# facebookresearch/iris

Hardware: AMD Instinct MI355X
Metric: bake_shading throughput (shading samples/s: secondary rays traced and shaded) (higher is better)
Workload: dtype f32; 1 GPU; bake_shading train-view sequence (15 views evenly spaced among 32 cameras on a circle, one view per step), 1920x1080, SPP=128 per lobe, lobes=[0, 1, 2, 3, 4, 5, 6] (0=diffuse,1-6=specular), synthetic room seed=1 1000990 triangles, SLF H=256, Philox uniforms; pixels_per_view=2073600

## Files before the change

### include/iris_hip_debug.h

```cpp
#ifndef IRIS_HIP_DEBUG_H
#define IRIS_HIP_DEBUG_H

#include "iris_hip.h"

#ifdef __cplusplus
extern "C" {
#endif

IRIS_API int iris_debug_scene_create(const float *verts, int64_t nv, const int32_t *faces, int64_t nf, int device, int layout,
                            iris_scene **out);

enum { IRIS_BAKE_AUTO = 0, IRIS_BAKE_PIXEL_PER_WAVE = 1, IRIS_BAKE_TILE_SORTED = 2 };

IRIS_API int iris_debug_bake_diffuse(const iris_scene *, const iris_emitter *, const iris_slf *, const float *pos, const float *nrm,
                            int64_t P, int spp, const float *u2, uint64_t seed, uint32_t stream_id, const int32_t *pix_id,
                            float *Ld, int64_t *tri_next, int64_t *src_next, uint64_t *stats, int variant, void *workspace,
                            uint64_t workspace_bytes, iris_stream_t);
IRIS_API int iris_debug_bake_specular(const iris_scene *, const iris_emitter *, const iris_slf *, const float *pos, const float *nrm,
                             const float *wo, float roughness, int64_t P, int spp, const float *u2, uint64_t seed,
                             uint32_t stream_id, const int32_t *pix_id, float *Ls0, float *Ls1, int64_t *tri_next, int64_t *src_next,
                             uint64_t *stats, int variant, void *workspace, uint64_t workspace_bytes, iris_stream_t);

IRIS_API int iris_debug_set(const char *key, long long value);
IRIS_API int iris_debug_ngp_encode(const iris_ngp *, const float *position, int64_t N, uint32_t *feat, iris_stream_t);
IRIS_API const char *iris_debug_build_flags(void);
IRIS_API const char *iris_debug_source_hash(void);

#ifdef __cplusplus
}
#endif
#endif
```

### iris_amd/_lib.py

```python
import ctypes as C
import os

import torch

_HERE = os.path.dirname(os.path.abspath(__file__))
LIB_PATH = os.environ.get("IRIS_HIP_LIB") or os.path.join(_HERE, "libiris_hip.so")

BVH_DEFAULT, BVH4_F32, BVH4_Q8 = 0, 1, 3
BAKE_AUTO, BAKE_PIXEL_PER_WAVE, BAKE_TILE_SORTED = 0, 1, 2


class IrisError(RuntimeError):
    pass


class SceneInfo(C.Structure):
    _fields_ = [("n_vertices", C.c_int64), ("n_triangles", C.c_int64), ("layout", C.c_int32), ("n_nodes", C.c_int32),
                ("node_bytes", C.c_int32), ("tri_bytes", C.c_int32), ("depth", C.c_int32), ("n_leaf_records", C.c_int32),
                ("sah_cost", C.c_float), ("build_seconds", C.c_float)]


_P, _I64, _I32, _F, _D, _U64, _U32 = C.c_void_p, C.c_int64, C.c_int, C.c_float, C.c_double, C.c_uint64, C.c_uint32

PROTOTYPES = {
# ... 10 lines not shown
    "iris_emitter_destroy": [_P],
    "iris_raygen_real": [_P, _P, _I32, _I32, _I32, _P, _P, _P, _P, _P],
    "iris_raygen_synthetic": [_F, _P, _I32, _I32, _I32, _P, _P, _P, _P, _P],
    "iris_intersect": [_P, _P, _P, _I64, _P, _P, _P, _P, _P, _P],
    "iris_sample_diffuse": [_P, _P, _I64, _P, _P, _P, _P],
    "iris_sample_specular": [_P, _P, _P, _F, _I64, _P, _P, _P, _P, _P],
    "iris_sample_specular_v": [_P, _P, _P, _P, _I64, _P, _P, _P, _P, _P],
    "iris_slf_lookup": [_P, _P, _I64, _P, _P, _P],
    "iris_eval_emitter": [_P, _P, _P, _P, _P, _F, _I64, _P, _P, _P, _P],
    "iris_bake_workspace_bytes": [_I64, _I32, _I32],
    "iris_bake_diffuse": [_P, _P, _P, _P, _P, _I64, _I32, _P, _U64, _U32, _P, _P, _P, _P, _U64, _P],
    "iris_bake_specular": [_P, _P, _P, _P, _P, _P, _F, _I64, _I32, _P, _U64, _U32, _P, _P, _P, _P, _P, _U64, _P],
    "iris_debug_bake_diffuse": [_P, _P, _P, _P, _P, _I64, _I32, _P, _U64, _U32, _P, _P, _P, _P, _P, _I32, _P, _U64, _P],
    "iris_debug_bake_specular": [_P, _P, _P, _P, _P, _P, _F, _I64, _I32, _P, _U64, _U32, _P, _P, _P, _P, _P, _P, _I32, _P, _U64, _P],
    "iris_debug_set": [C.c_char_p, C.c_longlong],
    "iris_debug_build_flags": [],
    "iris_debug_source_hash": [],
    "iris_bake_view": [_P, _P, _P, _P, _P, _P, _P, _I64, _I32, _P, _P, _P, _U64, _P, _P, _P, _U64, _P],
    "iris_lerp_specular": [_P, _P, _I64, _I32, _P, _P],
    "iris_unstripe_maps": [_P, _I32, _I32, _I64, _I32, _I32, _I32, _P, _P],
    "iris_get_normal_space": [_P, _I64, _P, _P],
    "iris_double_sided": [_P, _P, _I64, _P],
    "iris_angle2xyz": [_P, _P, _I64, _P, _P],
    "iris_ggx_terms": [_I32, _P, _P, _P, _I64, _P, _P, _P],
    "iris_philox_u2": [_U64, _U64, _U32, _I64, _P, _P],
    "iris_ngp_n_params": [],
    "iris_ngp_create": [_P, _I64, C.c_double, C.c_double, C.c_int, _P],
    "iris_ngp_forward": [_P, _P, _I64, _P, _P, _P, _P],
    "iris_ngp_set_params_dev": [_P, _P, _I64, _P],
    "iris_ngp_backward_workspace_bytes": [_I64],
# ... 168 lines not shown
```

### iris_amd/bake_shading.py

```python
import math
import os
import time

import torch

from . import _lib as L
from .utils.path_tracing import ray_intersect

SPP_DIFFUSE = 256
SPPS_SPECULAR = [64, 128, 128, 128, 128, 128]
N_ROUGHNESS = 6


def roughness_levels():
    return torch.linspace(0.02, 1.0, N_ROUGHNESS)


def _common(scene, emitter, position, normal, spp, u2, pix_id, want_tri):
    position = L.require_gpu(position, torch.float32, "position").reshape(-1, 3)
    normal = L.require_gpu(normal, torch.float32, "normal").reshape(-1, 3)
    P = position.shape[0]
    dev = position.device
    if u2 is not None:
        u2 = L.require_gpu(u2, torch.float32, "u2").reshape(-1, 2)
# ... 68 lines not shown
    levels = roughness_levels().tolist()
    if stream_ids is None:
        stream_ids = [0 if r is None else 1 + min(range(N_ROUGHNESS), key=lambda k: abs(levels[k] - float(r))) for r in roughness]
    outs0 = [torch.empty(P, 3, device=dev, dtype=torch.float32) for _ in range(n)]
    outs1 = [None if roughness[l] is None else torch.empty(P, 3, device=dev, dtype=torch.float32) for l in range(n)]
    rough = (C.c_float * n)(*[-1.0 if r is None else float(r) for r in roughness])
    spp_a = (C.c_int32 * n)(*[int(s) for s in spps])
    sid = (C.c_uint32 * n)(*[int(s) for s in stream_ids])
    p0 = (C.c_void_p * n)(*[t.data_ptr() for t in outs0])
    p1 = (C.c_void_p * n)(*[None if t is None else t.data_ptr() for t in outs1])
    ws, ws_bytes = _workspace(P, 1, True, L.BAKE_AUTO, dev)
    with torch.cuda.device(dev):
        L.check(L.lib().iris_bake_view(scene.handle, emitter.handle(dev), emitter.slf.handle(dev), L.ptr(position), L.ptr(normal), L.ptr(wo), L.ptr(pix_id),
                                       P, n, rough, spp_a, sid, int(seed), p0, p1, L.ptr(ws), ws_bytes, L.stream()))
    return [outs0[l] if roughness[l] is None else (outs0[l], outs1[l]) for l in range(n)]


def view_seed(seed, im_id):
    return (int(seed) + int(im_id) * 0x9E3779B97F4A7C15) & 0xFFFFFFFFFFFFFFFF


class LobeStreams:

    def __init__(self, device, n=3, emitter=None):
        self.main = torch.cuda.current_stream(device)
        if emitter is not None:
            emitter.handle(device); emitter.slf.handle(device)
        self.side = [torch.cuda.Stream(device=device) for _ in range(n)] if n > 1 else []
        self.k = 0

# ... 253 lines not shown
```

### iris_amd/csrc/iris_bake.h

```cpp
#pragma once
#include "iris_tile.h"

namespace iris {

struct BakeArgs {
    SceneDev sc; EmitDev em; SlfDev slf;
    const float* pos; const float* nrm; const float* wo;
    const float* u2; const int32_t* pix_id;
    int64_t P; int spp; uint64_t seed; uint32_t stream_id; float rough;
    float* out0; float* out1; int64_t* tri_next;
    int64_t* src_next;
    unsigned long long* stats;
    uint32_t* stack_ovf;
    float4* scratch;
    unsigned int* tile_counter;
    int tile_px;
};

#ifndef IRIS_TILE_RAYS
#define IRIS_TILE_RAYS 5120
#endif
constexpr int kTileRays = IRIS_TILE_RAYS;

__device__ __forceinline__ void reduce_geometry(int spp, int& lpp, int& ppw, int& rounds) {
// ... 143 lines not shown
        if (pvalid && sl == 0) {
            st3(a.out0 + p * 3, mk3(a0x * inv_spp, a0y * inv_spp, a0z * inv_spp));
            if (SPEC) st3(a.out1 + p * 3, mk3(a1x * inv_spp, a1y * inv_spp, a1z * inv_spp));
        }
    }
    flush_stats<COUNT>(a, ts, n_rays);
}

#ifndef IRIS_TILE_WAVES
#define IRIS_TILE_WAVES 7
#endif
#ifndef IRIS_TILE_STACK
#define IRIS_TILE_STACK 12
#endif

template <bool SPEC, bool COUNT, int LAYOUT, int TILE_STACK>
__device__ __forceinline__ void tile_body(const BakeArgs& a, int64_t p0, int np, float4* res, uint16_t* s_sorted, uint32_t* s_stack, int* s_chunk,
                                          uint32_t* ovf, TraceStats& ts, uint32_t& n_rays) {
    const int tid = threadIdx.x, lane = tid & 63, wave = tid >> 6;
    const int spp = a.spp;
    float2* res_g = reinterpret_cast<float2*>(res + kTileRays);
    int lpp, ppw, rounds;
    reduce_geometry(spp, lpp, ppw, rounds);
    const int sub = lane / lpp, sl = lane - sub * lpp;
    const float inv_spp = 1.0f / (float)spp;
    const int nr = np * spp;
    const bool resolve = !a.em.emit_ord && !a.tri_next;
    const bool skip_dead = dead_samples_skippable(a);

    const uint32_t spp_m = spp > 1 ? (uint32_t)(0x100000000ull / (uint64_t)(uint32_t)spp) + 1u : 0u;
    auto div_spp = [&](int r) -> int { return spp > 1 ? (int)__umulhi((uint32_t)r, spp_m) : r; };

    constexpr int kFrameOff = (kTileRays + 2 * 256 * 4) / 4, kFramePx = (TILE_STACK * kBlock - kFrameOff) / 6;
    float* s_frames = reinterpret_cast<float*>(s_stack) + kFrameOff;
    const bool frames = np <= kFramePx;
    if (frames) {
        for (int pl = tid; pl < np; pl += kBlock) {
            f3 t, b;
            normal_space(ld3(a.nrm + (p0 + pl) * 3), t, b);
            float* f = s_frames + pl * 6;
            f[0] = t.x; f[1] = t.y; f[2] = t.z; f[3] = b.x; f[4] = b.y; f[5] = b.z;
        }
        __syncthreads();
    }

    tile_sort_trace<LAYOUT, COUNT, kTileRays, TILE_STACK, true, SPEC && !COUNT>(
        a.sc, nr, s_sorted, s_stack, s_chunk, ovf, ts,
        [&](int r) -> uint32_t {
            const int pl = div_spp(r), s = r - pl * spp;
            const int64_t p = p0 + pl;
            const f3 n = ld3(a.nrm + p * 3), w = SPEC ? ld3(a.wo + p * 3) : mk3(0.f, 0.f, 1.f);
            const uint64_t base = (uint64_t)(a.pix_id ? (int64_t)a.pix_id[p] : p) * (uint64_t)spp;
            f3 t, b;
            if (frames) { const float* f = s_frames + pl * 6; t = mk3(f[0], f[1], f[2]); b = mk3(f[3], f[4], f[5]); }
            else normal_space(n, t, b);
            f3 wi; float g0, g1;
            sample_lobe<SPEC>(a, p, s, n, w, t, b, base, wi, g0, g1);
            if (SPEC) res_g[r] = make_float2(g1, g0);
            const bool dead = SPEC && !COUNT && skip_dead && g0 == 0.f && g1 == 0.f;
            res[r] = dead ? make_float4(0.f, 0.f, __int_as_float(resolve ? 0 : -1), __int_as_float(resolve ? -2 : 0)) : make_float4(wi.x, wi.y, wi.z, 0.f);
            return dead ? kDeadRay : dir_bin(wi);
        },
        [&](int r, f3& o, f3& d) {
            const int64_t p = p0 + div_spp(r);
            o = ld3(a.pos + p * 3);
            const float4 qa = res[r];
            d = mk3(qa.x, qa.y, qa.z);
        },
        [&](f3& o, f3& d) { o = mk3(o.x + kRayEps * d.x, o.y + kRayEps * d.y, o.z + kRayEps * d.z); },
        [&](int r, const Hit& h) {
            if (resolve) {
                float4 q = make_float4(0.f, 0.f, 0.f, __int_as_float(-2));
                if (h.slot >= 0) {
                    const float4* tr = a.sc.tris + (int64_t)h.slot * 4;
                    const float4 tx = tr[0], ty = tr[1], tz = tr[2];
                    const float ow = tr[3].x;
                    const f3 pn = hit_position(h, mk3(tx.x, ty.x, tz.x), mk3(tx.y, ty.y, tz.y), mk3(tx.z, ty.z, tz.z));
                    q = make_float4(pn.x, pn.y, pn.z, ow);
                }
                res[r] = q;
            } else
            res[r] = make_float4(h.u, h.v, __int_as_float(h.slot), 0.f);
            if (COUNT) n_rays++; }
        );

    const int n_groups = (np + ppw - 1) / ppw;
    IRIS_PHASE_BEGIN();
    for (int g = wave; g < n_groups; g += kBlock / 64) {
        const int pl = g * ppw + sub;
        const bool pvalid = pl < np;
        float a0x = 0.f, a0y = 0.f, a0z = 0.f, a1x = 0.f, a1y = 0.f, a1z = 0.f;
        if (resolve) {
            for (int rr = 0; rr < rounds; rr += 2) {
                const int s0 = rr * 64 + sl, s1 = s0 + 64;
                const bool ok0 = pvalid && s0 < spp, ok1 = pvalid && rr + 1 < rounds && s1 < spp;
                float4 q0 = make_float4(0.f, 0.f, 0.f, __int_as_float(-2)), q1 = q0;
                float2 w0 = make_float2(0.f, 0.f), w1 = w0;
                if (ok0) { q0 = res[pl * spp + s0]; if (SPEC) w0 = res_g[pl * spp + s0]; }
                if (ok1) { q1 = res[pl * spp + s1]; if (SPEC) w1 = res_g[pl * spp + s1]; }
                const int o0 = __float_as_int(q0.w), o1 = __float_as_int(q1.w);
                int j0 = -1, j1 = -1;
                if (o0 == -1) j0 = slf_index(a.slf, mk3(q0.x, q0.y, q0.z));
                if (o1 == -1) j1 = slf_index(a.slf, mk3(q1.x, q1.y, q1.z));
                float4 r0 = make_float4(0.f, 0.f, 0.f, 0.f), r1 = r0;
                if (o0 >= 0 || j0 >= 0) r0 = *(o0 >= 0 ? a.em.radiance + o0 : a.slf.radiance + j0);
                if (o1 >= 0 || j1 >= 0) r1 = *(o1 >= 0 ? a.em.radiance + o1 : a.slf.radiance + j1);
                if (ok0) {
                    const float z = o0 >= 0 ? -0.f : 0.f;
                    const f3 Le = mk3(z + r0.x, z + r0.y, z + r0.z);
                    if (a.src_next) a.src_next[(p0 + pl) * spp + s0] = o0 >= 0 ? -2 - o0 : j0;
                    if (SPEC) { a0x += Le.x * w0.y; a0y += Le.y * w0.y; a0z += Le.z * w0.y; a1x += Le.x * w0.x; a1y += Le.y * w0.x; a1z += Le.z * w0.x; }
                    else { a0x += Le.x; a0y += Le.y; a0z += Le.z; }
                }
                if (ok1) {
                    const float z = o1 >= 0 ? -0.f : 0.f;
                    const f3 Le = mk3(z + r1.x, z + r1.y, z + r1.z);
                    if (a.src_next) a.src_next[(p0 + pl) * spp + s1] = o1 >= 0 ? -2 - o1 : j1;
                    if (SPEC) { a0x += Le.x * w1.y; a0y += Le.y * w1.y; a0z += Le.z * w1.y; a1x += Le.x * w1.x; a1y += Le.y * w1.x; a1z += Le.z * w1.x; }
                    else { a0x += Le.x; a0y += Le.y; a0z += Le.z; }
                }
            }
        } else
        for (int rr = 0; rr < rounds; ++rr) {
            const int s = rr * 64 + sl;
            if (pvalid && s < spp) {
                const float4 qa = res[pl * spp + s];
                Hit h; h.u = qa.x; h.v = qa.y; h.slot = __float_as_int(qa.z); h.t = 0.f; h.id = 0;
                f3 pn = mk3(0.f, 0.f, 0.f);
                int64_t tri = -1;
                int ord_rec = -1;
                if (h.slot >= 0) {
                    const float4* tr = a.sc.tris + (int64_t)h.slot * 4;
                    const float4 tx = tr[0], ty = tr[1], tz = tr[2];
                    if (!a.em.emit_ord) ord_rec = __float_as_int(tr[3].x);
                    pn = hit_position(h, mk3(tx.x, ty.x, tz.x), mk3(tx.y, ty.y, tz.y), mk3(tx.z, ty.z, tz.z));
                    tri = __float_as_int(tx.w);
                }
                if (a.tri_next) a.tri_next[(p0 + pl) * spp + s] = tri;
                float epdf; bool vn; int src;
                const f3 Le = eval_emitter1(a.em, a.slf, pn, tri, true, 1.0f, 0.0f, epdf, vn, src, ord_rec);
                if (a.src_next) a.src_next[(p0 + pl) * spp + s] = src;
                if (SPEC) {
                    const float2 qb = res_g[pl * spp + s];
                    a0x += Le.x * qb.y; a0y += Le.y * qb.y; a0z += Le.z * qb.y;
                    a1x += Le.x * qb.x; a1y += Le.y * qb.x; a1z += Le.z * qb.x;
                } else { a0x += Le.x; a0y += Le.y; a0z += Le.z; }
            }
        }
        for (int m = 1; m < lpp; m <<= 1) {
            a0x += __shfl_xor(a0x, m); a0y += __shfl_xor(a0y, m); a0z += __shfl_xor(a0z, m);
            if (SPEC) { a1x += __shfl_xor(a1x, m); a1y += __shfl_xor(a1y, m); a1z += __shfl_xor(a1z, m); }
        }
        if (pvalid && sl == 0) {
            const int64_t p = p0 + pl;
            st3(a.out0 + p * 3, mk3(a0x * inv_spp, a0y * inv_spp, a0z * inv_spp));
            if (SPEC) st3(a.out1 + p * 3, mk3(a1x * inv_spp, a1y * inv_spp, a1z * inv_spp));
        }
    }
    IRIS_PHASE_MARK(3);
}

constexpr int kTileChunk = 64;
__device__ __forceinline__ long long claim_tile(unsigned int* counters, long long n_tiles) {
    constexpr int kChunk = kTileChunk;
    const long long n_chunks = (n_tiles + kChunk - 1) / kChunk;
    for (int k = 0; k < 8; ++k) {
        const int x = ((int)blockIdx.x + k) & 7;
        const long long per = (n_chunks + 7 - x) / 8;
        for (;;) {
            const unsigned int c = atomicAdd(counters + x, 1u);
            const long long ch = (long long)(c / kChunk);
            if (ch >= per) break;
            const long long t = (ch * 8 + x) * kChunk + (c % kChunk);
            if (t < n_tiles) return t;
// ... 32 lines not shown
constexpr int kMaxLobes = 8;
struct ViewLobe { float rough; int spp; uint32_t stream_id; int spec; int tile_px; int tiles_per_span; float* out0; float* out1; };
struct ViewArgs {
    BakeArgs base;
    int n_lobes;
    int span_px;
    long long n_tiles;
    ViewLobe lobe[kMaxLobes];
};

template <int LAYOUT>
__global__ __launch_bounds__(kBlock, IRIS_TILE_WAVES) void bake_view_kernel(ViewArgs v) {
    constexpr int kTileStack = IRIS_TILE_STACK;
    __shared__ uint16_t s_sorted[kTileRays];
    __shared__ uint32_t s_stack[kTileStack * kBlock];
    __shared__ int s_tile, s_chunk;
    static_assert(kTileStack * kBlock * 4 >= kTileRays + 2 * 256 * 4, "stack region too small to alias the sort keys");
    const int tid = threadIdx.x;
    float4* res = v.base.scratch + (size_t)blockIdx.x * kTileRays * 2;
    uint32_t* ovf = v.base.stack_ovf + (size_t)blockIdx.x * (kStackCapacity - kTileStack) * kBlock;
    for (;;) {
        __syncthreads();
        if (tid == 0) { s_tile = (int)claim_tile(v.base.tile_counter, v.n_tiles); s_chunk = 0; }
        (s_stack + kTileRays / 4)[tid] = 0;
        __syncthreads();
        const long long vt = s_tile;
        if (vt >= v.n_tiles) break;
        const long long g = vt / kTileChunk, q = g >> 3;
        const int j = (int)(vt % kTileChunk), l = (int)(q % v.n_lobes);
        const int64_t span0 = ((q / v.n_lobes) * 8 + (g & 7)) * (int64_t)v.span_px;
        const int64_t p0 = span0 + (int64_t)j * v.lobe[l].tile_px;
        if (j >= v.lobe[l].tiles_per_span || p0 >= v.base.P) continue;
        const int np = (int)min((int64_t)v.lobe[l].tile_px, min(v.base.P, span0 + v.span_px) - p0);
        BakeArgs a = v.base;
        a.spp = v.lobe[l].spp; a.rough = v.lobe[l].rough; a.stream_id = v.lobe[l].stream_id; a.tile_px = v.lobe[l].tile_px;
        a.out0 = v.lobe[l].out0; a.out1 = v.lobe[l].out1; a.u2 = nullptr; a.tri_next = nullptr; a.src_next = nullptr;
        TraceStats ts; uint32_t n_rays = 0;
        if (v.lobe[l].spec) tile_body<true, false, LAYOUT, kTileStack>(a, p0, np, res, s_sorted, s_stack, &s_chunk, ovf, ts, n_rays);
        else tile_body<false, false, LAYOUT, kTileStack>(a, p0, np, res, s_sorted, s_stack, &s_chunk, ovf, ts, n_rays);
    }
}

}
```

### iris_amd/csrc/iris_hip.hip

```cpp
#include <hip/hip_runtime.h>

#include <chrono>
#include <cmath>
#include <cstdio>
#include <cstring>
#include <atomic>
#include <cstdlib>
#include <memory>
#include <mutex>
#include <string>
#include <vector>

#include "../../include/iris_hip.h"
#include "../../include/iris_hip_debug.h"
#include "bvh_build.h"
#include "iris_device.h"
#include "iris_trace.h"
#include "iris_bake.h"
#include "iris_pt.h"
#include "iris_cache.h"
#include "iris_denoise.h"
#include "iris_ngp.h"
#include "iris_prop.h"
#include "iris_crf.h"
// ... 23 lines not shown
    DevBuf(DevBuf&& o) noexcept : p(o.p) { o.p = nullptr; }
    DevBuf& operator=(DevBuf&& o) noexcept { std::swap(p, o.p); return *this; }
    ~DevBuf() { if (p) (void)hipFree(p); }
    hipError_t alloc(size_t bytes) { return hipMalloc(&p, bytes); }
    hipError_t upload(const void* host, size_t bytes) { return hipMemcpy(p, host, bytes, hipMemcpyHostToDevice); }
};
struct DevEvent {
    hipEvent_t ev = nullptr;
    DevEvent() = default;
    DevEvent(DevEvent&& o) noexcept : ev(o.ev) { o.ev = nullptr; }
    DevEvent& operator=(DevEvent&& o) noexcept { std::swap(ev, o.ev); return *this; }
    ~DevEvent() { if (ev) (void)hipEventDestroy(ev); }
    hipError_t create() { return hipEventCreateWithFlags(&ev, hipEventDisableTiming); }
};

static long long g_opt_bvh_tri_cost_x100 = -1, g_opt_bvh_max_leaf = -1, g_opt_phase_min = -1, g_opt_tile_target_rays = -1, g_opt_tiles_per_block = -1, g_opt_pt_tile_min = -1, g_opt_bvh_presplit_x10 = -1, g_opt_joint_max_rays = -1, g_opt_prop_bwd_targets = -1, g_opt_prop_lds_members = -1;
extern "C" IRIS_API int iris_debug_set(const char* key, long long value) {
    if (!key) return fail(IRIS_ERR_ARG, "iris_debug_set: null key");
    const std::string k(key);
    if (k == "bvh_max_leaf") g_opt_bvh_max_leaf = value;
    else if (k == "bvh_tri_cost_x100") g_opt_bvh_tri_cost_x100 = value;
    else if (k == "bvh_presplit_x10") g_opt_bvh_presplit_x10 = value;
    else if (k == "phase_min") g_opt_phase_min = value;
    else if (k == "tile_target_rays") g_opt_tile_target_rays = value;
    else if (k == "tiles_per_block") g_opt_tiles_per_block = value;
    else if (k == "pt_tile_min") g_opt_pt_tile_min = value;
    else if (k == "joint_max_rays") g_opt_joint_max_rays = value;
    else if (k == "prop_bwd_targets") g_opt_prop_bwd_targets = value;
    else if (k == "prop_lds_members") g_opt_prop_lds_members = value;
    else return fail(IRIS_ERR_ARG, "iris_debug_set: unknown option " + k);
    return IRIS_OK;
}
extern "C" IRIS_API const char* iris_version(void) { return "iris_hip 0.1 (gfx950)"; }
#ifndef IRIS_NO_FUSED_RECORDS
#define IRIS_NO_FUSED_RECORDS 0
#endif
#ifndef IRIS_BUILD_FLAGS
#define IRIS_BUILD_FLAGS "unknown"
#endif
extern "C" IRIS_API const char* iris_debug_build_flags(void) { return IRIS_BUILD_FLAGS; }
#ifndef IRIS_SOURCE_HASH
#define IRIS_SOURCE_HASH "unknown"
#endif
extern "C" IRIS_API const char* iris_debug_source_hash(void) { return IRIS_SOURCE_HASH; }
// ... 1010 lines not shown
    if (em->fused.size() >= 2) { em->retired.push_back(std::move(em->fused.front())); em->fused.erase(em->fused.begin()); }
    int prev = 0;
    if (hipGetDevice(&prev) != hipSuccess || hipSetDevice(sc->device) != hipSuccess) { (void)hipGetLastError(); return nullptr; }
    DevBuf d; DevEvent ev;
    const int64_t n_rec = (int64_t)sc->dev.n_tris + 1;
    bool ok = d.alloc((size_t)n_rec * kLeafRecordBytes) == hipSuccess && ev.create() == hipSuccess;
    if (ok) {
        hipLaunchKernelGGL(fuse_ord_kernel, dim3(grid_for(n_rec, 256, 4096)), dim3(256), 0, st, sc->dev.tris, em->dev.emit_ord, n_rec, (float4*)d.p);
        ok = hipGetLastError() == hipSuccess && hipEventRecord(ev.ev, st) == hipSuccess;
    }
    (void)hipSetDevice(prev);
    if (!ok) { (void)hipGetLastError(); return nullptr; }
    em->fused.push_back({sc->uid, std::move(d), std::move(ev), false});
    return (const float4*)em->fused.back().d_tris.p;
}
extern "C" IRIS_API int iris_bake_view(const iris_scene* sc, const iris_emitter* em, const iris_slf* slf, const float* pos, const float* nrm,
                              const float* wo, const int32_t* pix_id, int64_t P, int n_lobes, const float* roughness, const int32_t* spp,
                              const uint32_t* stream_ids, uint64_t seed, float* const* out0, float* const* out1, void* workspace,
                              uint64_t workspace_bytes, iris_stream_t stream) {
    if (!sc || !em || !slf || P < 0 || n_lobes < 1 || n_lobes > kMaxLobes || !roughness || !spp || !stream_ids || !out0 || !out1 ||
        (P > 0 && (!pos || !nrm || !wo)))
        return fail(IRIS_ERR_ARG, "iris_bake_view: bad arguments");
    if (em->dev.nf != sc->info.n_triangles)
        return fail(IRIS_ERR_ARG, "iris_bake_view: the emitter tables were built for a mesh with a different number of triangles than the scene");
    if (P == 0) return IRIS_OK;
    const uint64_t need = iris_bake_workspace_bytes(P, 1, 1);
    if (!workspace || workspace_bytes < need) return fail(IRIS_ERR_ARG, "iris_bake_view: workspace of iris_bake_workspace_bytes() bytes required");
    ViewArgs v{};
    v.base.sc = sc->dev; v.base.em = em->dev; v.base.slf = slf->dev;
    if (const float4* ft = fused_tris(sc, em, (hipStream_t)stream)) { v.base.sc.tris = ft; v.base.em.emit_ord = nullptr; }
    v.base.pos = pos; v.base.nrm = nrm; v.base.wo = wo; v.base.pix_id = pix_id; v.base.P = P; v.base.seed = seed;
    v.base.tile_counter = (unsigned int*)workspace;
    v.base.scratch = (float4*)((char*)workspace + 256);
    v.base.stack_ovf = (uint32_t*)((char*)workspace + need - stack_ovf_bytes());
    v.n_lobes = n_lobes;
    const int blocks = bake_grid_blocks();
    long long t = 0;
    int tile_px_min = kTileRays;
    for (int l = 0; l < n_lobes; ++l) {
        if (spp[l] < 1 || spp[l] > kTileRays) return fail(IRIS_ERR_ARG, "iris_bake_view: spp must be in [1, iris_bake_tile_max_spp()]");
        if (!out0[l] || (roughness[l] >= 0.f && !out1[l])) return fail(IRIS_ERR_ARG, "iris_bake_view: null output");
        int tile_px = tile_pixels(spp[l]);
        const int64_t even = (P * n_lobes + (int64_t)blocks * 4 - 1) / ((int64_t)blocks * 4);
        if (even < tile_px) tile_px = (int)std::max<int64_t>(even, std::min(tile_px, 16));
        if (tile_px < 1) tile_px = 1;
        v.lobe[l].rough = roughness[l]; v.lobe[l].spp = spp[l]; v.lobe[l].stream_id = stream_ids[l]; v.lobe[l].spec = roughness[l] >= 0.f ? 1 : 0;
        v.lobe[l].tile_px = tile_px; v.lobe[l].out0 = out0[l]; v.lobe[l].out1 = out1[l];
        tile_px_min = std::min(tile_px_min, tile_px);
        t += (P + tile_px - 1) / tile_px;
    }
    v.span_px = kTileChunk * tile_px_min;
    for (int l = 0; l < n_lobes; ++l) v.lobe[l].tiles_per_span = (v.span_px + v.lobe[l].tile_px - 1) / v.lobe[l].tile_px;
    const long long n_spans = (P + v.span_px - 1) / v.span_px;
    hipStream_t st = (hipStream_t)stream;
    v.n_tiles = ((n_spans + 7) / 8) * 8 * n_lobes * kTileChunk;
    HIP_TRY(hipMemsetAsync(workspace, 0, 256, st));
    const int grid = (int)std::min<long long>(blocks, t);
    with_layout(v.base.sc, [&](auto t) { hipLaunchKernelGGL(bake_view_kernel<decltype(t)::layout>, dim3(grid), dim3(kBlock), 0, st, v); });
    HIP_TRY(hipGetLastError());
    return IRIS_OK;
}
extern "C" IRIS_API int iris_bake_diffuse(const iris_scene* sc, const iris_emitter* em, const iris_slf* slf, const float* pos, const float* nrm,
                                 int64_t P, int spp, const float* u2, uint64_t seed, uint32_t stream_id, const int32_t* pix_id,
                                 float* Ld, int64_t* tri_next, void* workspace, uint64_t workspace_bytes, iris_stream_t stream) {
    return bake_launch(false, sc, em, slf, pos, nrm, nullptr, -1.f, P, spp, u2, seed, stream_id, pix_id, Ld, nullptr, tri_next, nullptr, nullptr,
                       IRIS_BAKE_AUTO, workspace, workspace_bytes, stream);
}
extern "C" IRIS_API int iris_bake_specular(const iris_scene* sc, const iris_emitter* em, const iris_slf* slf, const float* pos, const float* nrm,
                                  const float* wo, float roughness, int64_t P, int spp, const float* u2, uint64_t seed,
                                  uint32_t stream_id, const int32_t* pix_id, float* Ls0, float* Ls1, int64_t* tri_next,
// ... 403 lines not shown
```

### iris_amd/csrc/iris_tile.h

```cpp
#pragma once
#include "iris_trace.h"

namespace iris {

#ifndef IRIS_PRIO_A
#define IRIS_PRIO_A 0
#endif
#ifndef IRIS_PRIO_C
#define IRIS_PRIO_C 3
#endif
#ifndef IRIS_PRIO_D
#define IRIS_PRIO_D 0
#endif

__device__ __forceinline__ uint32_t dir_bin(f3 d) {
    const float ax = fabsf(d.x), ay = fabsf(d.y), az = fabsf(d.z);
    const float inv = __builtin_amdgcn_rcpf(ax + ay + az + 1e-30f);
    const float a = ax * inv, b = ay * inv;
    const float v = b * __builtin_amdgcn_rcpf(1.f - a + 1e-30f);
    const int iu = min(7, (int)(a * 8.f)), iv0 = min(3, (int)(v * 4.f));
    const int iv = (iu & 1) ? 3 - iv0 : iv0;
    const uint32_t oct = (d.x < 0.f ? 1u : 0u) | (d.y < 0.f ? 2u : 0u) | (d.z < 0.f ? 4u : 0u);
    return (oct << 5) | ((uint32_t)iu << 2) | (uint32_t)iv;
}

#ifdef IRIS_PHASE_TIMING
__device__ unsigned long long g_phase_cycles[8];
#define IRIS_PHASE_BEGIN() unsigned long long t_phase_ = clock64()
#define IRIS_PHASE_MARK(k) do { if (threadIdx.x == 0) { const unsigned long long t_ = clock64(); atomicAdd(&g_phase_cycles[k], t_ - t_phase_); t_phase_ = t_; } } while (0)
#else
#define IRIS_PHASE_BEGIN()
#define IRIS_PHASE_MARK(k)
#endif

constexpr uint32_t kDeadRay = 256u;
template <int LAYOUT, bool COUNT, int CAP, int TILE_STACK, bool GLOBAL_OVF, bool SKIP_DEAD = false, class PhaseA, class FetchRay, class Prepare, class Retire>
__device__ __forceinline__ void tile_sort_trace(const SceneDev& sc, int nr, uint16_t* s_sorted, uint32_t* s_stack, int* s_chunk, uint32_t* ovf,
                                                TraceStats& ts, PhaseA phase_a, FetchRay fetch_ray, Prepare prepare, Retire retire) {
    static_assert(TILE_STACK * kBlock * 4 >= CAP + 2 * 256 * 4, "stack region too small to alias the sort keys");
    static_assert(!SKIP_DEAD || CAP <= 32 * kBlock, "one bit per ray of a thread");
    uint8_t* s_keys = reinterpret_cast<uint8_t*>(s_stack);
    uint32_t* s_hist = s_stack + CAP / 4;
    uint32_t* s_cur = s_hist + 256;
    const int tid = threadIdx.x, lane = tid & 63, wave = tid >> 6;
    IRIS_PHASE_BEGIN();
    __builtin_amdgcn_s_setprio(IRIS_PRIO_A);
    uint32_t dead = 0;
    if (SKIP_DEAD) {
        uint32_t bit = 1u;
        for (int r = tid; r < nr; r += kBlock, bit <<= 1) {
            const uint32_t key = phase_a(r);
            if (key == kDeadRay) dead |= bit;
            else { s_keys[r] = (uint8_t)key; atomicAdd(&s_hist[key], 1u); }
        }
    } else
    for (int r = tid; r < nr; r += kBlock) {
        const uint32_t key = phase_a(r);
        s_keys[r] = (uint8_t)key;
        atomicAdd(&s_hist[key], 1u);
    }
    __syncthreads();
    IRIS_PHASE_MARK(0);
    if (wave == 0) {
        uint32_t c0 = s_hist[lane * 4], c1 = s_hist[lane * 4 + 1], c2 = s_hist[lane * 4 + 2], c3 = s_hist[lane * 4 + 3];
        uint32_t tot = c0 + c1 + c2 + c3, inc = tot;
        for (int m = 1; m < 64; m <<= 1) { uint32_t v = __shfl_up(inc, m); if (lane >= m) inc += v; }
        uint32_t ex = inc - tot;
        if (SKIP_DEAD) {
            const uint32_t first = (uint32_t)nr - (uint32_t)__builtin_amdgcn_readlane((int)inc, 63);
            ex += first;
            if (lane == 0) *s_chunk = (int)first;
        }
        s_cur[lane * 4] = ex; s_cur[lane * 4 + 1] = ex + c0; s_cur[lane * 4 + 2] = ex + c0 + c1; s_cur[lane * 4 + 3] = ex + c0 + c1 + c2;
    }
    __syncthreads();
    if (SKIP_DEAD) {
        for (int r = tid; r < nr; r += kBlock, dead >>= 1) {
            if (dead & 1u) continue;
            const uint32_t pos = atomicAdd(&s_cur[s_keys[r]], 1u);
            s_sorted[pos] = (uint16_t)r;
        }
    } else
    for (int r = tid; r < nr; r += kBlock) {
        const uint32_t pos = atomicAdd(&s_cur[s_keys[r]], 1u);
        s_sorted[pos] = (uint16_t)r;
    }
    __syncthreads();
    IRIS_PHASE_MARK(1);
    {
        int my_r = 0;
// ... 8 lines not shown
            fetch_ray(my_r, o, d);
            return true;
        };
        auto ret = [&](const Hit& h) { retire(my_r, h); };
        __builtin_amdgcn_s_setprio(IRIS_PRIO_C);
        uint32_t tid_c = threadIdx.x;
        asm volatile("" : "+v"(tid_c));
        SceneDev sc_c = sc;
        asm volatile("" : "+s"(sc_c.nodes), "+s"(sc_c.tris), "+s"(sc_c.oct_stride));
        trace_stream<LAYOUT, COUNT, TILE_STACK, GLOBAL_OVF>(sc_c, s_stack + tid_c, tid_c, ovf, &ts, fetch, prepare, ret);
        __builtin_amdgcn_s_setprio(IRIS_PRIO_D);
        IRIS_PHASE_MARK(4);
    }
    __syncthreads();
    IRIS_PHASE_MARK(2);
}

}
```

Measured before the change: 10280 Mrays/s.

## Compact live specular samples into slots and grow specular tiles by dead share

For specular lobes in the fused bake_view kernel, dead samples (zero GGX weights) are no longer given slots in the tile buffer. Live samples are compacted into slots through a per-wave ballot and prefix count, and a per-64-ray group mask maps sample indices back to those slots during shading. Because fewer slots are used, the host planner enlarges each specular tile according to a roughness-based dead-share table, up to twice the base size. If a tile ends up with more live samples than the buffer holds, the block reprocesses it as two half tiles. This is meant to cut per-tile overhead and raise the number of useful rays per tile, at the cost of overflow retries and extra indirection.

```diff
diff --git a/include/iris_hip_debug.h b/include/iris_hip_debug.h
--- a/include/iris_hip_debug.h
+++ b/include/iris_hip_debug.h
@@ -22,6 +22,8 @@
                              uint64_t *stats, int variant, void *workspace, uint64_t workspace_bytes, iris_stream_t);
 
 IRIS_API int iris_debug_set(const char *key, long long value);
+IRIS_API int iris_debug_bake_view_plan(int64_t P, int n_lobes, const float *roughness, const int32_t *spp, int blocks, int32_t *tile_px,
+                              int32_t *tiles_per_span, int32_t *span_px, int64_t *n_tiles, uint64_t *slab_bytes);
 IRIS_API int iris_debug_ngp_encode(const iris_ngp *, const float *position, int64_t N, uint32_t *feat, iris_stream_t);
 IRIS_API const char *iris_debug_build_flags(void);
 IRIS_API const char *iris_debug_source_hash(void);
diff --git a/iris_amd/_lib.py b/iris_amd/_lib.py
--- a/iris_amd/_lib.py
+++ b/iris_amd/_lib.py
@@ -48,6 +48,7 @@
     "iris_debug_bake_diffuse": [_P, _P, _P, _P, _P, _I64, _I32, _P, _U64, _U32, _P, _P, _P, _P, _P, _I32, _P, _U64, _P],
     "iris_debug_bake_specular": [_P, _P, _P, _P, _P, _P, _F, _I64, _I32, _P, _U64, _U32, _P, _P, _P, _P, _P, _P, _I32, _P, _U64, _P],
     "iris_debug_set": [C.c_char_p, C.c_longlong],
+    "iris_debug_bake_view_plan": [_I64, _I32, _P, _P, _I32, _P, _P, _P, _P, _P],
     "iris_debug_build_flags": [],
     "iris_debug_source_hash": [],
     "iris_bake_view": [_P, _P, _P, _P, _P, _P, _P, _I64, _I32, _P, _P, _P, _U64, _P, _P, _P, _U64, _P],
diff --git a/iris_amd/bake_shading.py b/iris_amd/bake_shading.py
--- a/iris_amd/bake_shading.py
+++ b/iris_amd/bake_shading.py
@@ -106,6 +106,17 @@
         L.check(L.lib().iris_bake_view(scene.handle, emitter.handle(dev), emitter.slf.handle(dev), L.ptr(position), L.ptr(normal), L.ptr(wo), L.ptr(pix_id),
                                        P, n, rough, spp_a, sid, int(seed), p0, p1, L.ptr(ws), ws_bytes, L.stream()))
     return [outs0[l] if roughness[l] is None else (outs0[l], outs1[l]) for l in range(n)]
+
+
+def view_tile_plan(P, roughness, spps, blocks=0):
+    import ctypes as C
+    n = len(roughness)
+    rough = (C.c_float * n)(*[-1.0 if r is None else float(r) for r in roughness])
+    spp_a = (C.c_int32 * n)(*[int(s) for s in spps])
+    tile_px, tps = (C.c_int32 * n)(), (C.c_int32 * n)()
+    span, n_tiles, slab = C.c_int32(), C.c_int64(), C.c_uint64()
+    L.check(L.lib().iris_debug_bake_view_plan(int(P), n, rough, spp_a, int(blocks), tile_px, tps, C.byref(span), C.byref(n_tiles), C.byref(slab)))
+    return {"tile_px": list(tile_px), "tiles_per_span": list(tps), "span_px": span.value, "n_tiles": n_tiles.value, "slab_bytes": slab.value}
 
 
 def view_seed(seed, im_id):
diff --git a/iris_amd/csrc/iris_bake.h b/iris_amd/csrc/iris_bake.h
--- a/iris_amd/csrc/iris_bake.h
+++ b/iris_amd/csrc/iris_bake.h
@@ -181,9 +181,11 @@
 #define IRIS_TILE_STACK 12
 #endif
 
-template <bool SPEC, bool COUNT, int LAYOUT, int TILE_STACK>
-__device__ __forceinline__ void tile_body(const BakeArgs& a, int64_t p0, int np, float4* res, uint16_t* s_sorted, uint32_t* s_stack, int* s_chunk,
-                                          uint32_t* ovf, TraceStats& ts, uint32_t& n_rays) {
+constexpr int kLiveTileSamples = 2 * kTileRays;
+template <bool SPEC, bool COUNT, int LAYOUT, int TILE_STACK, bool LIVE = false>
+__device__ __forceinline__ bool tile_body(const BakeArgs& a, int64_t p0, int np, float4* res, uint16_t* s_sorted, uint32_t* s_stack, int* s_chunk,
+                                          uint32_t* ovf, TraceStats& ts, uint32_t& n_rays, int* s_nlive = nullptr) {
+    static_assert(!LIVE || (SPEC && !COUNT), "live slots: specular production tiles only");
     const int tid = threadIdx.x, lane = tid & 63, wave = tid >> 6;
     const int spp = a.spp;
     float2* res_g = reinterpret_cast<float2*>(res + kTileRays);
@@ -193,7 +195,8 @@
     const float inv_spp = 1.0f / (float)spp;
     const int nr = np * spp;
     const bool resolve = !a.em.emit_ord && !a.tri_next;
-    const bool skip_dead = dead_samples_skippable(a);
+    const bool skip_dead = LIVE || dead_samples_skippable(a);
+    uint4* grp = reinterpret_cast<uint4*>(res_g + kTileRays);
 
     const uint32_t spp_m = spp > 1 ? (uint32_t)(0x100000000ull / (uint64_t)(uint32_t)spp) + 1u : 0u;
     auto div_spp = [&](int r) -> int { return spp > 1 ? (int)__umulhi((uint32_t)r, spp_m) : r; };
@@ -211,7 +214,8 @@
         __syncthreads();
     }
 
-    tile_sort_trace<LAYOUT, COUNT, kTileRays, TILE_STACK, true, SPEC && !COUNT>(
+    f3 wi_a; float g0_a = 0.f, g1_a = 0.f; int pl_a = 0;
+    const bool over = tile_sort_trace<LAYOUT, COUNT, kTileRays, TILE_STACK, true, SPEC && !COUNT && !LIVE, LIVE>(
         a.sc, nr, s_sorted, s_stack, s_chunk, ovf, ts,
         [&](int r) -> uint32_t {
             const int pl = div_spp(r), s = r - pl * spp;
@@ -223,12 +227,19 @@
             else normal_space(n, t, b);
             f3 wi; float g0, g1;
             sample_lobe<SPEC>(a, p, s, n, w, t, b, base, wi, g0, g1);
+            if constexpr (LIVE) { wi_a = wi; g0_a = g0; g1_a = g1; pl_a = pl; return g0 == 0.f && g1 == 0.f ? kDeadRay : dir_bin(wi); }
             if (SPEC) res_g[r] = make_float2(g1, g0);
             const bool dead = SPEC && !COUNT && skip_dead && g0 == 0.f && g1 == 0.f;
             res[r] = dead ? make_float4(0.f, 0.f, __int_as_float(resolve ? 0 : -1), __int_as_float(resolve ? -2 : 0)) : make_float4(wi.x, wi.y, wi.z, 0.f);
             return dead ? kDeadRay : dir_bin(wi);
         },
         [&](int r, f3& o, f3& d) {
+            if constexpr (LIVE) {
+                const float4 qa = res[r];
+                d = mk3(qa.x, qa.y, qa.z);
+                o = ld3(a.pos + (p0 + __float_as_int(qa.w)) * 3);
+                return;
+            }
             const int64_t p = p0 + div_spp(r);
             o = ld3(a.pos + p * 3);
             const float4 qa = res[r];
@@ -248,8 +259,19 @@
                 res[r] = q;
             } else
             res[r] = make_float4(h.u, h.v, __int_as_float(h.slot), 0.f);
-            if (COUNT) n_rays++; }
+            if (COUNT) n_rays++; },
+        s_nlive,
+        [&](int slot) { res_g[slot] = make_float2(g1_a, g0_a); res[slot] = make_float4(wi_a.x, wi_a.y, wi_a.z, __int_as_float(pl_a)); },
+        [&](int g, unsigned long long m, int first) { grp[g] = make_uint4((uint32_t)m, (uint32_t)(m >> 32), (uint32_t)first, 0u); }
         );
+    if (LIVE && over) return true;
+    auto live_slot = [&](int r) -> int {
+        const uint4 G = grp[r >> 6];
+        const unsigned long long m = ((unsigned long long)G.y << 32) | G.x;
+        const int bit = r & 63;
+        if (!((m >> bit) & 1ull)) return -1;
+        return (int)G.z + __popcll(m & ((1ull << bit) - 1ull));
+    };
 
     const int n_groups = (np + ppw - 1) / ppw;
     IRIS_PHASE_BEGIN();
@@ -260,11 +282,19 @@
         if (resolve) {
             for (int rr = 0; rr < rounds; rr += 2) {
                 const int s0 = rr * 64 + sl, s1 = s0 + 64;
-                const bool ok0 = pvalid && s0 < spp, ok1 = pvalid && rr + 1 < rounds && s1 < spp;
+                bool ok0 = pvalid && s0 < spp, ok1 = pvalid && rr + 1 < rounds && s1 < spp;
                 float4 q0 = make_float4(0.f, 0.f, 0.f, __int_as_float(-2)), q1 = q0;
                 float2 w0 = make_float2(0.f, 0.f), w1 = w0;
-                if (ok0) { q0 = res[pl * spp + s0]; if (SPEC) w0 = res_g[pl * spp + s0]; }
-                if (ok1) { q1 = res[pl * spp + s1]; if (SPEC) w1 = res_g[pl * spp + s1]; }
+                if constexpr (LIVE) {
+                    int i0 = -1, i1 = -1;
+                    if (ok0) { i0 = live_slot(pl * spp + s0); ok0 = i0 >= 0; }
+                    if (ok1) { i1 = live_slot(pl * spp + s1); ok1 = i1 >= 0; }
+                    if (ok0) { q0 = res[i0]; w0 = res_g[i0]; }
+                    if (ok1) { q1 = res[i1]; w1 = res_g[i1]; }
+                } else {
+                    if (ok0) { q0 = res[pl * spp + s0]; if (SPEC) w0 = res_g[pl * spp + s0]; }
+                    if (ok1) { q1 = res[pl * spp + s1]; if (SPEC) w1 = res_g[pl * spp + s1]; }
+                }
                 const int o0 = __float_as_int(q0.w), o1 = __float_as_int(q1.w);
                 int j0 = -1, j1 = -1;
                 if (o0 == -1) j0 = slf_index(a.slf, mk3(q0.x, q0.y, q0.z));
@@ -291,7 +321,9 @@
         for (int rr = 0; rr < rounds; ++rr) {
             const int s = rr * 64 + sl;
             if (pvalid && s < spp) {
-                const float4 qa = res[pl * spp + s];
+                int i = 0;
+                if constexpr (LIVE) { i = live_slot(pl * spp + s); if (i < 0) continue; }
+                const float4 qa = res[LIVE ? i : pl * spp + s];
                 Hit h; h.u = qa.x; h.v = qa.y; h.slot = __float_as_int(qa.z); h.t = 0.f; h.id = 0;
                 f3 pn = mk3(0.f, 0.f, 0.f);
                 int64_t tri = -1;
@@ -308,7 +340,7 @@
                 const f3 Le = eval_emitter1(a.em, a.slf, pn, tri, true, 1.0f, 0.0f, epdf, vn, src, ord_rec);
                 if (a.src_next) a.src_next[(p0 + pl) * spp + s] = src;
                 if (SPEC) {
-                    const float2 qb = res_g[pl * spp + s];
+                    const float2 qb = res_g[LIVE ? i : pl * spp + s];
                     a0x += Le.x * qb.y; a0y += Le.y * qb.y; a0z += Le.z * qb.y;
                     a1x += Le.x * qb.x; a1y += Le.y * qb.x; a1z += Le.z * qb.x;
                 } else { a0x += Le.x; a0y += Le.y; a0z += Le.z; }
@@ -325,6 +357,7 @@
         }
     }
     IRIS_PHASE_MARK(3);
+    return false;
 }
 
 constexpr int kTileChunk = 64;
@@ -387,31 +420,39 @@
     constexpr int kTileStack = IRIS_TILE_STACK;
     __shared__ uint16_t s_sorted[kTileRays];
     __shared__ uint32_t s_stack[kTileStack * kBlock];
-    __shared__ int s_tile, s_chunk;
+    __shared__ int s_tile, s_chunk, s_nlive, s_pend;
     static_assert(kTileStack * kBlock * 4 >= kTileRays + 2 * 256 * 4, "stack region too small to alias the sort keys");
     const int tid = threadIdx.x;
+    if (tid == 0) s_pend = 0;
     float4* res = v.base.scratch + (size_t)blockIdx.x * kTileRays * 2;
     uint32_t* ovf = v.base.stack_ovf + (size_t)blockIdx.x * (kStackCapacity - kTileStack) * kBlock;
     for (;;) {
         __syncthreads();
-        if (tid == 0) { s_tile = (int)claim_tile(v.base.tile_counter, v.n_tiles); s_chunk = 0; }
+        if (tid == 0) { if (s_pend == 0) s_tile = (int)claim_tile(v.base.tile_counter, v.n_tiles); s_chunk = 0; s_nlive = 0; }
         (s_stack + kTileRays / 4)[tid] = 0;
         __syncthreads();
         const long long vt = s_tile;
         if (vt >= v.n_tiles) break;
+        const int pend = s_pend;
         const long long g = vt / kTileChunk, q = g >> 3;
         const int j = (int)(vt % kTileChunk), l = (int)(q % v.n_lobes);
         const int64_t span0 = ((q / v.n_lobes) * 8 + (g & 7)) * (int64_t)v.span_px;
-        const int64_t p0 = span0 + (int64_t)j * v.lobe[l].tile_px;
+        int64_t p0 = span0 + (int64_t)j * v.lobe[l].tile_px;
         if (j >= v.lobe[l].tiles_per_span || p0 >= v.base.P) continue;
-        const int np = (int)min((int64_t)v.lobe[l].tile_px, min(v.base.P, span0 + v.span_px) - p0);
+        int np = (int)min((int64_t)v.lobe[l].tile_px, min(v.base.P, span0 + v.span_px) - p0);
+        if (pend) {
+            const int h = (np + 1) >> 1;
+            if (pend == 2) np = h; else { p0 += h; np -= h; }
+        }
         BakeArgs a = v.base;
         a.spp = v.lobe[l].spp; a.rough = v.lobe[l].rough; a.stream_id = v.lobe[l].stream_id; a.tile_px = v.lobe[l].tile_px;
         a.out0 = v.lobe[l].out0; a.out1 = v.lobe[l].out1; a.u2 = nullptr; a.tri_next = nullptr; a.src_next = nullptr;
         TraceStats ts; uint32_t n_rays = 0;
-        if (v.lobe[l].spec) tile_body<true, false, LAYOUT, kTileStack>(a, p0, np, res, s_sorted, s_stack, &s_chunk, ovf, ts, n_rays);
+        bool over = false;
+        if (v.lobe[l].spec) over = tile_body<true, false, LAYOUT, kTileStack, true>(a, p0, np, res, s_sorted, s_stack, &s_chunk, ovf, ts, n_rays, &s_nlive);
         else tile_body<false, false, LAYOUT, kTileStack>(a, p0, np, res, s_sorted, s_stack, &s_chunk, ovf, ts, n_rays);
-    }
-}
-
-}
+        if (tid == 0) s_pend = over ? 2 : (pend ? pend - 1 : 0);
+    }
+}
+
+}
diff --git a/iris_amd/csrc/iris_hip.hip b/iris_amd/csrc/iris_hip.hip
--- a/iris_amd/csrc/iris_hip.hip
+++ b/iris_amd/csrc/iris_hip.hip
@@ -61,7 +61,7 @@
     hipError_t create() { return hipEventCreateWithFlags(&ev, hipEventDisableTiming); }
 };
 
-static long long g_opt_bvh_tri_cost_x100 = -1, g_opt_bvh_max_leaf = -1, g_opt_phase_min = -1, g_opt_tile_target_rays = -1, g_opt_tiles_per_block = -1, g_opt_pt_tile_min = -1, g_opt_bvh_presplit_x10 = -1, g_opt_joint_max_rays = -1, g_opt_prop_bwd_targets = -1, g_opt_prop_lds_members = -1;
+static long long g_opt_bvh_tri_cost_x100 = -1, g_opt_bvh_max_leaf = -1, g_opt_phase_min = -1, g_opt_tile_target_rays = -1, g_opt_tiles_per_block = -1, g_opt_pt_tile_min = -1, g_opt_bvh_presplit_x10 = -1, g_opt_joint_max_rays = -1, g_opt_prop_bwd_targets = -1, g_opt_prop_lds_members = -1, g_opt_tile_live_samples = -1, g_opt_tile_live_comp_x100 = -1;
 extern "C" IRIS_API int iris_debug_set(const char* key, long long value) {
     if (!key) return fail(IRIS_ERR_ARG, "iris_debug_set: null key");
     const std::string k(key);
@@ -75,6 +75,8 @@
     else if (k == "joint_max_rays") g_opt_joint_max_rays = value;
     else if (k == "prop_bwd_targets") g_opt_prop_bwd_targets = value;
     else if (k == "prop_lds_members") g_opt_prop_lds_members = value;
+    else if (k == "tile_live_samples") g_opt_tile_live_samples = value;
+    else if (k == "tile_live_comp_x100") g_opt_tile_live_comp_x100 = value;
     else return fail(IRIS_ERR_ARG, "iris_debug_set: unknown option " + k);
     return IRIS_OK;
 }
@@ -1115,6 +1117,54 @@
     em->fused.push_back({sc->uid, std::move(d), std::move(ev), false});
     return (const float4*)em->fused.back().d_tris.p;
 }
+constexpr int kLiveCompDefault = 100;
+static float dead_share(float rough) {
+    static const float kr[6] = {0.02f, 0.216f, 0.412f, 0.608f, 0.804f, 1.0f}, kd[6] = {0.f, 0.009f, 0.087f, 0.233f, 0.378f, 0.5f};
+    if (!(rough > kr[0])) return 0.f;
+    for (int i = 1; i < 6; ++i) if (rough <= kr[i]) return kd[i - 1] + (kd[i] - kd[i - 1]) * (rough - kr[i - 1]) / (kr[i] - kr[i - 1]);
+    return kd[5];
+}
+static int live_tile_cap_px(int spp) {
+    const int half = kTileRays / spp;
+    return std::max(1, half <= 1 ? 1 : std::min(2 * half, kLiveTileSamples / spp));
+}
+struct ViewPlan { int tile_px[kMaxLobes], tiles_per_span[kMaxLobes], span_px; long long n_tiles, real_tiles; };
+static ViewPlan view_plan(int64_t P, int n_lobes, const float* roughness, const int32_t* spp, int blocks) {
+    ViewPlan pl{};
+    int tile_px_min = kTileRays;
+    for (int l = 0; l < n_lobes; ++l) {
+        int tile_px = tile_pixels(spp[l]);
+        const bool spec = roughness[l] >= 0.f;
+        if (spec) {
+            const float comp = (float)(g_opt_tile_live_comp_x100 >= 0 ? std::min<long long>(100, g_opt_tile_live_comp_x100) : kLiveCompDefault) * 0.01f;
+            const int grown = (int)((float)(tile_px * spp[l]) / (1.f - comp * dead_share(roughness[l]))) / spp[l];
+            tile_px = std::min(std::max(tile_px, grown), std::max(tile_px, live_tile_cap_px(spp[l])));
+        }
+        const int64_t even = (P * n_lobes + (int64_t)blocks * 4 - 1) / ((int64_t)blocks * 4);
+        if (even < tile_px) tile_px = (int)std::max<int64_t>(even, std::min(tile_px, 16));
+        if (spec && g_opt_tile_live_samples > 0) tile_px = (int)std::min<long long>(live_tile_cap_px(spp[l]), std::max<long long>(1, g_opt_tile_live_samples / spp[l]));
+        if (tile_px < 1) tile_px = 1;
+        pl.tile_px[l] = tile_px;
+        tile_px_min = std::min(tile_px_min, tile_px);
+        pl.real_tiles += (P + tile_px - 1) / tile_px;
+    }
+    pl.span_px = kTileChunk * tile_px_min;
+    for (int l = 0; l < n_lobes; ++l) pl.tiles_per_span[l] = (pl.span_px + pl.tile_px[l] - 1) / pl.tile_px[l];
+    const long long n_spans = (P + pl.span_px - 1) / pl.span_px;
+    pl.n_tiles = ((n_spans + 7) / 8) * 8 * n_lobes * kTileChunk;
+    return pl;
+}
+extern "C" IRIS_API int iris_debug_bake_view_plan(int64_t P, int n_lobes, const float* roughness, const int32_t* spp, int blocks, int32_t* tile_px,
+                                                  int32_t* tiles_per_span, int32_t* span_px, int64_t* n_tiles, uint64_t* slab_bytes) {
+    if (P < 0 || n_lobes < 1 || n_lobes > kMaxLobes || !roughness || !spp || !tile_px || !tiles_per_span || !span_px || !n_tiles || !slab_bytes)
+        return fail(IRIS_ERR_ARG, "iris_debug_bake_view_plan: bad arguments");
+    for (int l = 0; l < n_lobes; ++l) if (spp[l] < 1 || spp[l] > kTileRays) return fail(IRIS_ERR_ARG, "iris_debug_bake_view_plan: spp must be in [1, iris_bake_tile_max_spp()]");
+    const ViewPlan pl = view_plan(P, n_lobes, roughness, spp, blocks > 0 ? blocks : bake_grid_blocks());
+    for (int l = 0; l < n_lobes; ++l) { tile_px[l] = pl.tile_px[l]; tiles_per_span[l] = pl.tiles_per_span[l]; }
+    *span_px = pl.span_px; *n_tiles = pl.n_tiles;
+    *slab_bytes = (uint64_t)kTileRays * 2 * sizeof(float4);
+    return IRIS_OK;
+}
 extern "C" IRIS_API int iris_bake_view(const iris_scene* sc, const iris_emitter* em, const iris_slf* slf, const float* pos, const float* nrm,
                               const float* wo, const int32_t* pix_id, int64_t P, int n_lobes, const float* roughness, const int32_t* spp,
                               const uint32_t* stream_ids, uint64_t seed, float* const* out0, float* const* out1, void* workspace,
@@ -1135,26 +1185,20 @@
     v.base.scratch = (float4*)((char*)workspace + 256);
     v.base.stack_ovf = (uint32_t*)((char*)workspace + need - stack_ovf_bytes());
     v.n_lobes = n_lobes;
-    const int blocks = bake_grid_blocks();
-    long long t = 0;
-    int tile_px_min = kTileRays;
     for (int l = 0; l < n_lobes; ++l) {
         if (spp[l] < 1 || spp[l] > kTileRays) return fail(IRIS_ERR_ARG, "iris_bake_view: spp must be in [1, iris_bake_tile_max_spp()]");
         if (!out0[l] || (roughness[l] >= 0.f && !out1[l])) return fail(IRIS_ERR_ARG, "iris_bake_view: null output");
-        int tile_px = tile_pixels(spp[l]);
-        const int64_t even = (P * n_lobes + (int64_t)blocks * 4 - 1) / ((int64_t)blocks * 4);
-        if (even < tile_px) tile_px = (int)std::max<int64_t>(even, std::min(tile_px, 16));
-        if (tile_px < 1) tile_px = 1;
+    }
+    const int blocks = bake_grid_blocks();
+    const ViewPlan plan = view_plan(P, n_lobes, roughness, spp, blocks);
+    for (int l = 0; l < n_lobes; ++l) {
         v.lobe[l].rough = roughness[l]; v.lobe[l].spp = spp[l]; v.lobe[l].stream_id = stream_ids[l]; v.lobe[l].spec = roughness[l] >= 0.f ? 1 : 0;
-        v.lobe[l].tile_px = tile_px; v.lobe[l].out0 = out0[l]; v.lobe[l].out1 = out1[l];
-        tile_px_min = std::min(tile_px_min, tile_px);
-        t += (P + tile_px - 1) / tile_px;
-    }
-    v.span_px = kTileChunk * tile_px_min;
-    for (int l = 0; l < n_lobes; ++l) v.lobe[l].tiles_per_span = (v.span_px + v.lobe[l].tile_px - 1) / v.lobe[l].tile_px;
-    const long long n_spans = (P + v.span_px - 1) / v.span_px;
+        v.lobe[l].tile_px = plan.tile_px[l]; v.lobe[l].tiles_per_span = plan.tiles_per_span[l]; v.lobe[l].out0 = out0[l]; v.lobe[l].out1 = out1[l];
+    }
+    v.span_px = plan.span_px;
+    const long long t = plan.real_tiles;
     hipStream_t st = (hipStream_t)stream;
-    v.n_tiles = ((n_spans + 7) / 8) * 8 * n_lobes * kTileChunk;
+    v.n_tiles = plan.n_tiles;
     HIP_TRY(hipMemsetAsync(workspace, 0, 256, st));
     const int grid = (int)std::min<long long>(blocks, t);
     with_layout(v.base.sc, [&](auto t) { hipLaunchKernelGGL(bake_view_kernel<decltype(t)::layout>, dim3(grid), dim3(kBlock), 0, st, v); });
diff --git a/iris_amd/csrc/iris_tile.h b/iris_amd/csrc/iris_tile.h
--- a/iris_amd/csrc/iris_tile.h
+++ b/iris_amd/csrc/iris_tile.h
@@ -34,11 +34,14 @@
 #endif
 
 constexpr uint32_t kDeadRay = 256u;
-template <int LAYOUT, bool COUNT, int CAP, int TILE_STACK, bool GLOBAL_OVF, bool SKIP_DEAD = false, class PhaseA, class FetchRay, class Prepare, class Retire>
-__device__ __forceinline__ void tile_sort_trace(const SceneDev& sc, int nr, uint16_t* s_sorted, uint32_t* s_stack, int* s_chunk, uint32_t* ovf,
-                                                TraceStats& ts, PhaseA phase_a, FetchRay fetch_ray, Prepare prepare, Retire retire) {
+template <int LAYOUT, bool COUNT, int CAP, int TILE_STACK, bool GLOBAL_OVF, bool SKIP_DEAD = false, bool LIVE = false, class PhaseA, class FetchRay, class Prepare, class Retire,
+          class Park = int, class Group = int>
+__device__ __forceinline__ bool tile_sort_trace(const SceneDev& sc, int nr, uint16_t* s_sorted, uint32_t* s_stack, int* s_chunk, uint32_t* ovf,
+                                                TraceStats& ts, PhaseA phase_a, FetchRay fetch_ray, Prepare prepare, Retire retire,
+                                                int* s_nlive = nullptr, Park park = Park(), Group group = Group()) {
     static_assert(TILE_STACK * kBlock * 4 >= CAP + 2 * 256 * 4, "stack region too small to alias the sort keys");
     static_assert(!SKIP_DEAD || CAP <= 32 * kBlock, "one bit per ray of a thread");
+    static_assert(!(LIVE && SKIP_DEAD), "LIVE keeps dead rays out of the slots altogether");
     uint8_t* s_keys = reinterpret_cast<uint8_t*>(s_stack);
     uint32_t* s_hist = s_stack + CAP / 4;
     uint32_t* s_cur = s_hist + 256;
@@ -46,6 +49,22 @@
     IRIS_PHASE_BEGIN();
     __builtin_amdgcn_s_setprio(IRIS_PRIO_A);
     uint32_t dead = 0;
+    int n_live = 0;
+    if constexpr (LIVE) {
+        for (int k0 = 0; k0 < nr; k0 += kBlock) {
+            const int r = k0 + tid;
+            uint32_t key = kDeadRay;
+            if (r < nr) key = phase_a(r);
+            const bool live = key != kDeadRay;
+            const unsigned long long m = __ballot(live);
+            int base = 0;
+            if (lane == 0) base = atomicAdd(s_nlive, __popcll(m));
+            base = __builtin_amdgcn_readfirstlane(base);
+            if (lane == 0) group(r >> 6, m, base);
+            const int slot = base + (int)__builtin_amdgcn_mbcnt_hi((uint32_t)(m >> 32), __builtin_amdgcn_mbcnt_lo((uint32_t)m, 0u));
+            if (live && slot < CAP) { park(slot); s_keys[slot] = (uint8_t)key; atomicAdd(&s_hist[key], 1u); }
+        }
+    } else
     if (SKIP_DEAD) {
         uint32_t bit = 1u;
         for (int r = tid; r < nr; r += kBlock, bit <<= 1) {
@@ -61,12 +80,17 @@
     }
     __syncthreads();
     IRIS_PHASE_MARK(0);
+    if constexpr (LIVE) {
+        n_live = *s_nlive;
+        if (n_live > CAP) return true;
+        nr = min(nr, CAP);
+    }
     if (wave == 0) {
         uint32_t c0 = s_hist[lane * 4], c1 = s_hist[lane * 4 + 1], c2 = s_hist[lane * 4 + 2], c3 = s_hist[lane * 4 + 3];
         uint32_t tot = c0 + c1 + c2 + c3, inc = tot;
         for (int m = 1; m < 64; m <<= 1) { uint32_t v = __shfl_up(inc, m); if (lane >= m) inc += v; }
         uint32_t ex = inc - tot;
-        if (SKIP_DEAD) {
+        if (SKIP_DEAD || LIVE) {
             const uint32_t first = (uint32_t)nr - (uint32_t)__builtin_amdgcn_readlane((int)inc, 63);
             ex += first;
             if (lane == 0) *s_chunk = (int)first;
@@ -74,6 +98,12 @@
         s_cur[lane * 4] = ex; s_cur[lane * 4 + 1] = ex + c0; s_cur[lane * 4 + 2] = ex + c0 + c1; s_cur[lane * 4 + 3] = ex + c0 + c1 + c2;
     }
     __syncthreads();
+    if constexpr (LIVE) {
+        for (int r = tid; r < n_live; r += kBlock) {
+            const uint32_t pos = atomicAdd(&s_cur[s_keys[r]], 1u);
+            s_sorted[pos] = (uint16_t)r;
+        }
+    } else
     if (SKIP_DEAD) {
         for (int r = tid; r < nr; r += kBlock, dead >>= 1) {
             if (dead & 1u) continue;
@@ -112,6 +142,7 @@
     }
     __syncthreads();
     IRIS_PHASE_MARK(2);
+    return false;
 }
 
 }
```

Result: no change. 10300 Mrays/s (median of 3 runs) (+0.1%).
